# levayz/diffusion_finetuning

Hardware: AMD Instinct MI355X
Metric: images/s SD1.5 LoRA rank-4 512^2 train step (higher is better)
Workload: dtype f16; 1 GPU; SD1.5 UNet-only LoRA rank=4, batch=4/GPU, 512^2 (64x64x4 latents), f16 storage/compute, fp32 accumulate + fp32 master LoRA, full train step (fwd+bwd+clip+AdamW); global_batch=4, parallelism=dp1, lora_params=1246464, overflow=False, hipgraph=True, conv_autotune=True, rccl_ranks=1

## Files before the change

diffusion_finetuning_amd/_native.py:

```python
import ctypes
import os
import threading

import torch

_LIB_PATH = os.environ.get("DFA_LIB_PATH") or os.path.join(os.path.dirname(os.path.abspath(__file__)), "lib", "liblora_hip.so")
_lib = None
_lock = threading.Lock()

ABI_VERSION = 9
PROF_KINDS = 18

_DTYPE_CODE = {torch.float32: 0, torch.float16: 1, torch.bfloat16: 2}

_vp, _i64, _i32, _f32 = ctypes.c_void_p, ctypes.c_int64, ctypes.c_int, ctypes.c_float


class GradProblem(ctypes.Structure):
    _fields_ = [
        ("S", _vp), ("P", _vp), ("out", _vp * 4),
        ("s_stride", _i64), ("p_stride", _i64), ("part_stride", _i64), ("M", _i64),
        ("C", _i32), ("r", _i32), ("rg", _i32), ("out_kn", _i32), ("n_blocks", _i32),
        ("scale", _f32),
    ]
# ... 83 lines not shown
    "lora_adamw_rows": (_i32, [_vp, _vp, _vp, _vp, _vp, _i64, _i32, _vp, _f32, _f32, _f32, _f32, _f32, _f32, _f32, _i32, _vp]),
    "ti_rows_grad": (_i32, [_vp, _vp, _i64, _i32, _vp, _i32, _vp, _i32, _i32, _vp]),
    "ti_rows_adamw_decay": (_i32, [_vp, _i64, _i32, _vp, _i32, _vp, _vp, _vp, _f32, _f32, _f32, _f32, _f32, _f32, _i32, _f32, _f32,
                                   _vp]),
    "geglu_linear_bwd": (_i32, [_vp, _vp, _vp, _vp, _vp, _i64, _i32, _i32, _i32, _vp]),
    "geglu_gate_fwd": (_i32, [_vp, _vp, _i64, _i32, _i32, _vp]),
    "geglu_gate_bwd": (_i32, [_vp, _vp, _vp, _i64, _i32, _i32, _vp]),
    "attn_split_heads": (_i32, [_vp, _vp, _i32, _i32, _i32, _i32, _i32, _i32, _vp]),
    "attn_merge_heads": (_i32, [_vp, _vp, _i32, _i32, _i32, _i32, _i32, _i32, _vp]),
    "attn_merge_heads_strided": (_i32, [_vp, _vp, _i32, _i32, _i32, _i32, _i32, _i64, _i64, _i64, _i32, _vp]),
    "group_norm_act_workspace_bytes": (_i64, [_i32, _i32, _i32, _i32, _i32, _i32]),
    "group_norm_act_plan": (_i32, [_i32, _i32, _i32, _i32, _i32, _i32]),
    "group_norm_act_fwd": (_i32, [_vp] * 8 + [_i32, _i32, _i32, _i32, _f32, _i32, _i32, _i32, _vp]),
    "group_norm_act_bwd": (_i32, [_vp] * 10 + [_i32, _i32, _i32, _i32, _i32, _i32, _i32, _vp]),
    "group_norm_act_bwd_res": (_i32, [_vp] * 11 + [_i32, _i32, _i32, _i32, _i32, _i32, _vp]),
    "residual_bias_add_supported": (_i32, [_i32, _i32, _i32, _i32]),
    "residual_bias_add": (_i32, [_vp] * 5 + [_i32, _i32, _i32, _i32, _vp]),
    "tokens_nchw_supported": (_i32, [_i32, _i32, _i32, _i32]),
    "tokens_to_nchw_add": (_i32, [_vp] * 3 + [_i32, _i32, _i32, _i32, _vp]),
    "nchw_to_tokens": (_i32, [_vp] * 2 + [_i32, _i32, _i32, _i32, _vp]),
    "time_proj_supported": (_i32, [_i32, _i32, _i32]),
    "time_proj_all": (_i32, [_vp] * 6 + [_i32, _i32, _i32, _i32, _vp]),
    "conv3x3_small_supported": (_i32, [_i32, _i32, _i32, _i32, _i32, _i32]),
    "conv3x3_small_workspace_bytes": (_i64, [_i32, _i32, _i32, _i32, _i32, _i32]),
    "conv3x3_small_plan": (_i32, [_i64, _i32, _i32, _i32]),
    "conv3x3_small_plan_channels": (_i32, [_i32, _i32, _i32]),
    "conv3x3_small_pack": (_i32, [_vp, _vp, _i32, _i32, _i32, _i32, _vp]),
    "conv3x3_small": (_i32, [_vp] * 5 + [_i64, _i32, _i32, _i32, _i32, _i32, _i32, _vp]),
    "conv3x3_large_supported": (_i32, [_i32, _i32, _i32, _i32, _i32, _i32]),
    "conv3x3_large_workspace_bytes": (_i64, [_i32, _i32, _i32, _i32, _i32, _i32]),
    "conv3x3_large_plan": (_i32, [_i64, _i32, _i32, _i32]),
    "conv3x3_large_plan_channels": (_i32, [_i32, _i32, _i32]),
    "conv3x3_large": (_i32, [_vp] * 5 + [_i64, _i32, _i32, _i32, _i32, _i32, _i32, _vp]),
    "add_layer_norm_max_channels": (_i32, []),
    "add_layer_norm_fwd": (_i32, [_vp] * 8 + [_i64, _i32, _f32, _i32, _vp]),
    "add_layer_norm_bwd": (_i32, [_vp] * 7 + [_i64, _i32, _i32, _vp]),
    "attn_ctx_supported": (_i32, [_i32, _i32, _i32, _i32, _i32, _i32]),
    "attn_ctx_fwd": (_i32, [_vp, _vp, _vp, _vp, _i32, _i32, _i32, _i32, _i32, _f32, _i32, _vp]),
    "attn_ctx_bwd_workspace_bytes": (_i64, [_i32, _i32, _i32, _i32, _i32]),
    "attn_ctx_fwd_strided": (_i32, [_vp, _vp, _vp, _vp, _i64, _i32, _i32, _i32, _i32, _i32, _f32, _i32, _vp]),
    "attn_ctx_bwd_strided": (_i32, [_vp] * 8 + [_i64, _i64, _i32, _i32, _i32, _i32, _i32, _f32, _i32, _vp]),
    "attn_flash_fwd_strided": (_i32, [_vp, _vp, _vp, _vp, _vp, _i64, _i32, _i32, _i32, _i32, _i32, _f32, _i32, _vp]),
    "attn_flash_bwd_strided": (_i32, [_vp] * 10 + [_i64, _i64, _i32, _i32, _i32, _i32, _i32, _f32, _i32, _vp]),
    "attn_ctx_bwd": (_i32, [_vp, _vp, _vp, _vp, _vp, _vp, _vp, _vp, _i32, _i32, _i32, _i32, _i32, _f32, _i32, _vp]),
    "attn_causal_supported": (_i32, [_i32, _i32, _i32, _i32, _i32]),
    "attn_causal_fwd_strided": (_i32, [_vp, _vp, _vp, _vp, _i64, _i32, _i32, _i32, _i32, _f32, _i32, _vp]),
    "attn_causal_bwd_workspace_bytes": (_i64, [_i32, _i32, _i32, _i32]),
    "attn_causal_bwd_strided": (_i32, [_vp] * 8 + [_i64, _i64, _i32, _i32, _i32, _i32, _f32, _i32, _vp]),
    "attn_flash_supported": (_i32, [_i32, _i32, _i32, _i32, _i32, _i32]),
    "attn_flash_fwd": (_i32, [_vp, _vp, _vp, _vp, _vp, _i32, _i32, _i32, _i32, _i32, _f32, _i32, _vp]),
    "attn_flash_bwd_workspace_bytes": (_i64, [_i32, _i32, _i32]),
    "attn_flash_bwd": (_i32, [_vp] * 10 + [_i32, _i32, _i32, _i32, _i32, _f32, _i32, _vp]),
    "attn_f32_supported": (_i32, [_i32, _i32, _i32, _i32, _i32]),
    "attn_f32_fwd": (_i32, [_vp, _vp, _vp, _vp, _vp, _i32, _i32, _i32, _i32, _i32, _f32, _vp]),
    "attn_f32_bwd_workspace_bytes": (_i64, [_i32, _i32, _i32]),
    "attn_f32_bwd": (_i32, [_vp] * 10 + [_i32, _i32, _i32, _i32, _i32, _f32, _vp]),
    "lora_distill_workspace_bytes": (_i64, [_i64, _i64]),
    "lora_distill_start": (_i32, [_vp, _i32, _i64, _i32, _i64, _vp, _vp]),
    "lora_distill_diff": (_i32, [_vp, _i32, _i64, _i32, _i32, _vp, _vp]),
    "lora_distill_rayleigh_ritz": (_i32, [_vp, _i32, _i32, _i32, ctypes.c_double, _i32, _vp, _vp]),
    "lora_distill_finalize": (_i32, [_vp, _i32, _i32, _f32, _i32, _vp, _vp, _vp]),
    "lora_quantile_clamp": (_i32, [_vp, _i64, _f32, _vp, _vp]),
    "lora_distill_wide_width": (_i32, [_i32]),
    "lora_distill_wide_workspace_bytes": (_i64, [_i64, _i64, _i32]),
    "lora_distill_wide_start": (_i32, [_vp, _i32, _i64, _i32, _i64, _vp, _vp]),
    "lora_distill_wide_diff": (_i32, [_vp, _i32, _i64, _i32, _i32, _i32, _vp, _vp]),
# ... 1153 lines not shown
def conv3x3_small(x, pack, bias, Cout: int):
    _require_device(x, pack, bias)
    N, Cin, H, W = x.shape
    code = dtype_code(x.dtype)
    nbytes = int(lib().conv3x3_small_workspace_bytes(N, Cin, Cout, H, W, code))
    ws = torch.empty(max(nbytes, 16) // 4, dtype=torch.float32, device=x.device)
    y = torch.empty((N, Cout, H, W), dtype=x.dtype, device=x.device)
    _check(lib().conv3x3_small(_ptr(x), _ptr(pack), _ptr(bias), _ptr(y), _ptr(ws), nbytes, N, Cin, Cout, H, W, code, _stream(x)),
           "conv3x3_small")
    return y


def conv3x3_large_supported(N: int, Cin: int, Cout: int, H: int, W: int, dtype) -> bool:
    return dtype in (torch.float16, torch.bfloat16) and bool(lib().conv3x3_large_supported(N, Cin, Cout, H, W, dtype_code(dtype)))


def conv3x3_large_plan(pixels: int, Cin: int, Cout: int, dtype) -> bool:
    return dtype in (torch.float16, torch.bfloat16) and bool(lib().conv3x3_large_plan(int(pixels), Cin, Cout, dtype_code(dtype)))


def conv3x3_large_plan_channels(Cin: int, Cout: int, dtype) -> bool:
    return dtype in (torch.float16, torch.bfloat16) and bool(lib().conv3x3_large_plan_channels(Cin, Cout, dtype_code(dtype)))


def conv3x3_large(x, pack, bias, Cout: int):
    _require_device(x, pack, bias)
    N, Cin, H, W = x.shape
    y = torch.empty((N, Cout, H, W), dtype=x.dtype, device=x.device)
    _check(lib().conv3x3_large(_ptr(x), _ptr(pack), _ptr(bias), _ptr(y), None, 0, N, Cin, Cout, H, W, dtype_code(x.dtype),
                               _stream(x)), "conv3x3_large")
    return y


def tokens_nchw_supported(N: int, C: int, HW: int, dtype) -> bool:
    return dtype in (torch.float16, torch.bfloat16) and bool(lib().tokens_nchw_supported(N, C, HW, dtype_code(dtype)))


def tokens_to_nchw_add(tok, res, shape):
    _require_device(tok, res)
    N, C, H, W = shape
    out = torch.empty(shape, dtype=tok.dtype, device=tok.device)
    _check(lib().tokens_to_nchw_add(_ptr(tok), _ptr(res), _ptr(out), N, C, H * W, dtype_code(tok.dtype), _stream(tok)),
           "tokens_to_nchw_add")
    return out


def nchw_to_tokens(x):
    _require_device(x)
    N, C, H, W = x.shape
    tok = torch.empty((N, H * W, C), dtype=x.dtype, device=x.device)
    _check(lib().nchw_to_tokens(_ptr(x), _ptr(tok), N, C, H * W, dtype_code(x.dtype), _stream(x)), "nchw_to_tokens")
    return tok


def add_layer_norm_supported(x) -> bool:
    C = x.shape[-1] if x.dim() else 0
    return (x.numel() > 0 and x.is_contiguous() and C % 8 == 0 and C <= lib().add_layer_norm_max_channels() and
            x.data_ptr() % 16 == 0)


def add_layer_norm_fwd(x, delta, gamma, beta, eps: float):
    _require_device(x, delta, gamma, beta)
    C = x.shape[-1]
    M = x.numel() // C
    h = None if delta is None else torch.empty_like(x)
    y = torch.empty_like(x)
# ... 262 lines not shown
```

diffusion_finetuning_amd/build_native.py:

```python
import hashlib
import os
import subprocess
import sys
from concurrent.futures import ThreadPoolExecutor

PKG_DIR = os.path.dirname(os.path.abspath(__file__))
CSRC = os.path.join(PKG_DIR, "csrc")
LIB_DIR = os.path.join(PKG_DIR, "lib")
LIB_PATH = os.path.join(LIB_DIR, "liblora_hip.so")
SOURCES = ["lora_gemm.hip", "lora_grad.hip", "ddpm_loss.hip", "optim.hip", "sandwich.hip", "norm.hip", "trunk_edges.hip", "time_proj.hip", "conv_small.hip", "conv_large.hip", "layer_norm.hip", "attn_ctx.hip", "attn_causal.hip", "attn_flash.hip", "attn_f32.hip", "embed.hip", "distill.hip", "distill_wide.hip", "prof.hip"]
HIPCC = os.environ.get("HIPCC", "/opt/rocm/bin/hipcc")
FLAGS = ["--offload-arch=gfx950", "-O3", "-std=c++17", "-fPIC", "-Wall", "-Wno-unused-function"]
SOURCE_FLAGS = {}


def _digest() -> str:
    h = hashlib.sha256()
    for name in sorted(os.listdir(CSRC)) + [os.path.join("..", "..", "include", "lora_hip.h")]:
        with open(os.path.join(CSRC, name), "rb") as f:
            h.update(name.encode())
            h.update(f.read())
    h.update(" ".join(FLAGS).encode())
    for name in sorted(SOURCE_FLAGS):
        h.update((name + " " + " ".join(SOURCE_FLAGS[name])).encode())
    return h.hexdigest()


def build(force: bool = False, verbose: bool = True, variant: str = "", defines=()) -> str:
    os.makedirs(LIB_DIR, exist_ok=True)
    lib_path = os.path.join(LIB_DIR, f"liblora_hip_{variant}.so") if variant else LIB_PATH
    obj_dir = os.path.join(LIB_DIR, f"obj_{variant}") if variant else LIB_DIR
    os.makedirs(obj_dir, exist_ok=True)
    stamp = os.path.join(LIB_DIR, f"liblora_hip_{variant}.stamp" if variant else "liblora_hip.stamp")
    digest = _digest() + (" " + " ".join(defines) if defines else "")
    if not force and os.path.exists(lib_path) and os.path.exists(stamp):
        with open(stamp) as f:
            if f.read().strip() == digest:
                return lib_path

    def compile_one(src: str) -> str:
        obj = os.path.join(obj_dir, src.replace(".hip", ".o"))
        cmd = [HIPCC, *FLAGS, *SOURCE_FLAGS.get(src, []), *defines, "-c", os.path.join(CSRC, src), "-o", obj]
        if verbose:
# ... 24 lines not shown
```

diffusion_finetuning_amd/conv.py:

```python
import torch
import torch.nn as nn
import torch.nn.functional as F
from torch.autograd.function import once_differentiable
from torch.utils.weak import WeakIdKeyDictionary

from . import _native as nat

ROUTES = ("auto", "hip", "large", "stock")

_FAMILY = {"hip": "small", "large": "large"}

_packs = WeakIdKeyDictionary()


def _key(weight):
    return (weight.data_ptr(), weight._version, weight.dtype, weight.device)


def _get_packs(weight):
    entry = _packs.get(weight)
    key = _key(weight)
    if entry is not None and entry[0] == key:
        return entry[1], entry[2]
    if torch.cuda.is_current_stream_capturing():
        return None
    w = weight.detach()
    entry = (key, nat.conv3x3_small_pack(w, False), nat.conv3x3_small_pack(w, True))
    _packs[weight] = entry
    return entry[1], entry[2]


def _weight_eligible(weight, bias) -> bool:
    if not weight.is_cuda or weight.dtype not in (torch.float16, torch.bfloat16) or weight.dim() != 4:
        return False
    if tuple(weight.shape[2:]) != (3, 3) or weight.shape[0] % 32 or weight.shape[1] % 32 or not weight.is_contiguous():
        return False
    if weight.data_ptr() % 16 or weight.requires_grad:
        return False
    if bias is not None and (bias.requires_grad or bias.dtype != weight.dtype or bias.device != weight.device or
                             bias.shape != weight.shape[:1] or not bias.is_contiguous()):
        return False
    return True


def _supported(x, weight, bias, family="small") -> bool:
    if not _weight_eligible(weight, bias):
        return False
    if x.dim() != 4 or x.dtype != weight.dtype or x.device != weight.device or x.shape[1] != weight.shape[1]:
        return False
    if x.numel() == 0 or not x.is_contiguous() or x.data_ptr() % 16:
        return False
    N, Cin, H, W = x.shape
    Cout = weight.shape[0]
    covers = nat.conv3x3_small_supported if family == "small" else nat.conv3x3_large_supported
    return covers(N, Cin, Cout, H, W, x.dtype) and covers(N, Cout, Cin, H, W, x.dtype)


def _run(family, x, pack, bias, Cout):
    return (nat.conv3x3_small if family == "small" else nat.conv3x3_large)(x, pack, bias, Cout)


# ... 18 lines not shown
    def backward(ctx, dy):
        if not ctx.needs_input_grad[0]:
            return (None,) * 7
        dy = dy.contiguous()
        if dy.data_ptr() % 16:
            dy = dy.clone()
        return (_run(ctx.bwd_family, dy, ctx.bwd_pack, None, ctx.cin),) + (None,) * 6


def conv3x3(x: torch.Tensor, weight: torch.Tensor, bias=None, route: str = "auto") -> torch.Tensor:
    if route not in ROUTES:
        raise ValueError(f"conv3x3: route must be one of {ROUTES}, got {route!r}")
    if route != "stock":
        fwd = bwd = None
        if route == "auto":
            if x.dim() == 4 and weight.dim() == 4 and x.is_cuda:
                N, Cin, H, W = x.shape
                fwd = _auto_family(N * H * W, Cin, weight.shape[0], x.dtype)
                bwd = _auto_family(N * H * W, weight.shape[0], Cin, x.dtype) if fwd is not None else None
                if bwd is None or not all(_supported(x, weight, bias, f) for f in {fwd, bwd}):
                    fwd = bwd = None
        elif _supported(x, weight, bias, _FAMILY[route]):
            fwd = bwd = _FAMILY[route]
        packs = _get_packs(weight) if fwd is not None else None
        if packs is not None:
            return _Conv3x3Fn.apply(x, weight, bias, packs[0], packs[1], fwd, bwd)
        if route != "auto":
            raise RuntimeError(f"conv3x3(route={route!r}): the HIP kernel does not cover this call (needs a frozen 16-bit 3×3 "
                               "weight with channel counts that are multiples of 32, an NCHW-contiguous x of the same dtype "
                               "from a 16-byte boundary, and a pack made before stream capture)")
    return F.conv2d(x, weight, bias, padding=1)


def prepack_conv3x3(module: nn.Module, route: str = "auto") -> int:
    if route not in ROUTES:
        raise ValueError(f"prepack_conv3x3: route must be one of {ROUTES}, got {route!r}")
    if route == "stock":
        return 0
    n = 0
    for m in module.modules():
        if type(m) is not nn.Conv2d or m.kernel_size != (3, 3) or m.stride != (1, 1) or m.padding != (1, 1):
            continue
        if m.dilation != (1, 1) or m.groups != 1 or not _weight_eligible(m.weight, m.bias):
            continue
        if route == "auto" and not (nat.conv3x3_small_plan_channels(m.weight.shape[1], m.weight.shape[0], m.weight.dtype) or
                                    nat.conv3x3_large_plan_channels(m.weight.shape[1], m.weight.shape[0], m.weight.dtype)):
            continue
        if _get_packs(m.weight) is not None:
            n += 1
    return n


def packed_bytes() -> int:
    return sum(e[1].numel() * e[1].element_size() + e[2].numel() * e[2].element_size() for e in _packs.values())
```

harness/unet.py:

```python
import math
from dataclasses import dataclass, field
from typing import List, Optional, Tuple

import torch
import torch.nn as nn
import torch.nn.functional as F
from torch.nn.attention import SDPBackend, sdpa_kernel


@dataclass
class UNetConfig:
    in_channels: int = 4
    out_channels: int = 4
    block_out_channels: Tuple[int, ...] = (320, 640, 1280, 1280)
    down_attention: Tuple[bool, ...] = (True, True, True, False)
    layers_per_block: int = 2
    num_heads: Tuple[int, ...] = (8, 8, 8, 8)
    cross_attention_dim: int = 768
    norm_groups: int = 32
    linear_projection: bool = False
    name: str = "sd15"


def sd15_config() -> UNetConfig:
# ... 38 lines not shown
    def forward(self, x):
        return self.linear_2(self.act(self.linear_1(x)))


def _fused_norms(x):
    return x.is_cuda and x.dtype in (torch.float16, torch.bfloat16)


def _norm_act(norm: nn.GroupNorm, x, act: bool, addend=None):
    from diffusion_finetuning_amd.norm import group_norm_act

    return group_norm_act(x, norm.num_groups, norm.weight, norm.bias, norm.eps, act, addend)


def _norm_act_res(norm: nn.GroupNorm, x, act: bool):
    from diffusion_finetuning_amd.norm import group_norm_act_res

    return group_norm_act_res(x, norm.num_groups, norm.weight, norm.bias, norm.eps, act)


def _norm_tokens(norm: nn.GroupNorm, x):
    from diffusion_finetuning_amd.norm import group_norm_tokens

    return group_norm_tokens(x, norm.num_groups, norm.weight, norm.bias, norm.eps)


def _tokens_to_nchw_add(tok, res):
    from diffusion_finetuning_amd.norm import tokens_to_nchw_add

    return tokens_to_nchw_add(tok, res)


CONV3X3_ROUTE = "auto"


def _conv3x3(x, weight, bias=None):
    from diffusion_finetuning_amd.conv import conv3x3

    return conv3x3(x, weight, bias, CONV3X3_ROUTE)


def _residual_bias_add(h, res, b1, b2=None):
    from diffusion_finetuning_amd.norm import residual_bias_add

    return residual_bias_add(h, res, b1, b2)


def _time_projections(temb, layers):
    from diffusion_finetuning_amd.time_proj import time_projections

    return time_projections(temb, layers)


def _layer_norm(norm: nn.LayerNorm, x):
    from diffusion_finetuning_amd import norm as dnorm

    return dnorm.layer_norm(x, norm.weight, norm.bias, norm.eps)


def _add_layer_norm(norm: nn.LayerNorm, x, delta):
    from diffusion_finetuning_amd import norm as dnorm

    return dnorm.add_layer_norm(x, delta, norm.weight, norm.bias, norm.eps)


class ResnetBlock2D(nn.Module):
# ... 139 lines not shown
        x = _norm_act(self.norm, x, False) if _fused_norms(x) else self.norm(x)
        if x.is_cuda and not self.linear_projection:
            x = F.linear(x.permute(0, 2, 3, 1).reshape(b, h * w, c), self.proj_in.weight.view(c, c), self.proj_in.bias)
            for blk in self.transformer_blocks:
                x = blk(x, context)
            x = F.linear(x, self.proj_out.weight.view(c, c), self.proj_out.bias)
            return x.view(b, h, w, c).permute(0, 3, 1, 2).contiguous() + res
        if self.linear_projection:
            x = self.proj_in(x.permute(0, 2, 3, 1).reshape(b, h * w, c))
        else:
            x = self.proj_in(x).permute(0, 2, 3, 1).reshape(b, h * w, c)
        for blk in self.transformer_blocks:
            x = blk(x, context)
        if self.linear_projection:
            x = self.proj_out(x).reshape(b, h, w, c).permute(0, 3, 1, 2).contiguous()
        else:
            x = self.proj_out(x.reshape(b, h, w, c).permute(0, 3, 1, 2))
        return x + res


class Downsample2D(nn.Module):
    def __init__(self, c):
        super().__init__()
        self.conv = nn.Conv2d(c, c, 3, stride=2, padding=1)

    def forward(self, x):
        return self.conv(x)


class Upsample2D(nn.Module):
    def __init__(self, c):
        super().__init__()
        self.conv = nn.Conv2d(c, c, 3, padding=1)

    def forward(self, x):
        x = F.interpolate(x, scale_factor=2.0, mode="nearest")
        if _fused_norms(x) and type(self.conv) is nn.Conv2d:
            return _conv3x3(x, self.conv.weight, self.conv.bias)
        return self.conv(x)


class DownBlock(nn.Module):
    def __init__(self, cin, cout, temb, layers, attn, heads, ctx, groups, linear_proj, add_down):
        super().__init__()
        self.attentions = nn.ModuleList(
            [Transformer2DModel(cout, heads, ctx, groups, linear_proj) for _ in range(layers)] if attn else []
        )
        self.resnets = nn.ModuleList([ResnetBlock2D(cin if i == 0 else cout, cout, temb, groups) for i in range(layers)])
        self.downsamplers = nn.ModuleList([Downsample2D(cout)]) if add_down else None

    def forward(self, x, temb, context, addends=None):
        outs = []
        for i, res in enumerate(self.resnets):
            x = res(x, temb, None if addends is None else addends[i])
            if len(self.attentions):
                x = self.attentions[i](x, context)
            outs.append(x)
        if self.downsamplers is not None:
            x = self.downsamplers[0](x)
            outs.append(x)
        return x, outs


class MidBlock(nn.Module):
    def __init__(self, c, temb, heads, ctx, groups, linear_proj):
        super().__init__()
        self.attentions = nn.ModuleList([Transformer2DModel(c, heads, ctx, groups, linear_proj)])
        self.resnets = nn.ModuleList([ResnetBlock2D(c, c, temb, groups), ResnetBlock2D(c, c, temb, groups)])
# ... 100 lines not shown
```

include/lora_hip.h:

```cpp
#ifndef LORA_HIP_H
#define LORA_HIP_H

#include <stdint.h>

#ifdef __cplusplus
extern "C" {
#endif

#define LORA_HIP_ABI_VERSION 9

enum lora_dtype { LORA_F32 = 0, LORA_F16 = 1, LORA_BF16 = 2 };

enum lora_status {
    LORA_OK = 0,
    LORA_E_BADARG = -1,
    LORA_E_RANK = -2,
    LORA_E_ALIGN = -3,
    LORA_E_LAUNCH = -4,
    LORA_E_UNSUPPORTED = -5
};

int lora_version(void);

const char* lora_status_string(int status);
// ... 202 lines not shown
                       int HW, int groups, int act, int channels_last, int dtype, void* stream);
int group_norm_act_bwd_res(const void* dy, const void* dh , const void* x, const void* addend ,
                           const void* gamma, const void* beta, const float* mean, const float* rstd, void* dx,
                           void* da , void* workspace, int N, int C, int HW, int groups, int act, int dtype,
                           void* stream);

int residual_bias_add_supported(int N, int C, int HW, int dtype);
int residual_bias_add(const void* h, const void* res, const void* b1, const void* b2 , void* out, int N, int C,
                      int HW, int dtype, void* stream);
int tokens_nchw_supported(int N, int C, int HW, int dtype);
int tokens_to_nchw_add(const void* tok, const void* res , void* out, int N, int C, int HW, int dtype,
                       void* stream);
int nchw_to_tokens(const void* x, void* tok, int N, int C, int HW, int dtype, void* stream);

int time_proj_supported(int N, int E, int dtype);
int time_proj_all(const void* t, const void* const* W, const void* const* b , const void* const* cb ,
                  const int* C, void* out, int L, int N, int E, int dtype, void* stream);

int conv3x3_small_supported(int N, int C_in, int C_out, int H, int W, int dtype);
int64_t conv3x3_small_workspace_bytes(int N, int C_in, int C_out, int H, int W, int dtype);
int conv3x3_small_plan(int64_t pixels, int C_in, int C_out, int dtype);
int conv3x3_small_plan_channels(int C_in, int C_out, int dtype);
int conv3x3_small_pack(const void* w, void* packed, int C_in, int C_out, int backward, int dtype, void* stream);
int conv3x3_small(const void* x, const void* wpack, const void* bias , void* y, void* workspace,
                  int64_t workspace_bytes, int N, int C_in, int C_out, int H, int W, int dtype, void* stream);

int conv3x3_large_supported(int N, int C_in, int C_out, int H, int W, int dtype);
int64_t conv3x3_large_workspace_bytes(int N, int C_in, int C_out, int H, int W, int dtype);
int conv3x3_large_plan(int64_t pixels, int C_in, int C_out, int dtype);
int conv3x3_large_plan_channels(int C_in, int C_out, int dtype);
int conv3x3_large(const void* x, const void* wpack, const void* bias , void* y, void* workspace ,
                  int64_t workspace_bytes, int N, int C_in, int C_out, int H, int W, int dtype, void* stream);

int add_layer_norm_max_channels(void);
int add_layer_norm_fwd(const void* x, const void* delta , const void* gamma, const void* beta,
                       void* h , void* y, float* mean, float* rstd, int64_t M, int C, float eps,
                       int dtype, void* stream);
int add_layer_norm_bwd(const void* dy, const void* dh , const void* h, const void* gamma, const float* mean,
                       const float* rstd, void* dx, int64_t M, int C, int dtype, void* stream);

int embed_rows_fwd(const float* table, const int64_t* ids, void* out, int64_t n, int D, int64_t V, int out_dtype, void* stream);
int embed_rows_bwd(const void* dE, const int64_t* ids, float* grad_table, unsigned char* active , int64_t n,
                   int D, int64_t V, int dtype, int accumulate, void* stream);
int lora_adamw_rows(float* param, const float* grad, float* exp_avg, float* exp_avg_sq, const unsigned char* active, int64_t V,
                    int D, const float* norm_in, float grad_mul, float max_norm, float lr, float beta1, float beta2, float eps,
                    float weight_decay, int step, void* stream);

#define LORA_TI_MAX_ROWS 64
int ti_rows_grad(const void* dE, const int64_t* ids, int64_t n, int D, const int64_t* slot_ids, int P, float* grad, int dtype,
                 int accumulate, void* stream);
int ti_rows_adamw_decay(float* table, int64_t V, int D, const int64_t* slot_ids, int P, const float* grad, float* exp_avg,
                        float* exp_avg_sq, float grad_mul, float lr, float beta1, float beta2, float eps, float weight_decay,
                        int step, float decay_lambda, float target_norm, void* stream);

int attn_ctx_supported(int B, int Tq, int Tk, int H, int d, int dtype);
int attn_ctx_fwd_strided(const void* Q, const void* K, const void* V, void* O, int64_t ldk, int B, int Tq, int Tk,
                         int H, int d, float scale, int dtype, void* stream);
int attn_ctx_bwd_strided(const void* Q, const void* K, const void* V, const void* dO, void* dQ, void* dK, void* dV,
                         void* workspace, int64_t ldk, int64_t ld_dk, int B, int Tq, int Tk, int H, int d,
                         float scale, int dtype, void* stream);
int attn_ctx_fwd(const void* Q, const void* K, const void* V, void* O, int B, int Tq, int Tk, int H, int d,
                 float scale, int dtype, void* stream);
int64_t attn_ctx_bwd_workspace_bytes(int B, int Tq, int Tk, int H, int d);
int attn_ctx_bwd(const void* Q, const void* K, const void* V, const void* dO, void* dQ, void* dK, void* dV,
                 void* workspace, int B, int Tq, int Tk, int H, int d, float scale, int dtype, void* stream);

// ... 67 lines not shown
```

Before: 203.2 images/s.

## Fuse nearest 2x upsample with following 3x3 conv via subpixel 2x2 weights

Adds a HIP kernel that computes nearest-upsample followed by a 3x3 conv directly from the low-resolution input. It uses four precombined 2x2 subpixel weight sets, which cuts MACs by about 2.25x and skips materialising the upsampled tensor. A matching backward kernel produces the input gradient at low resolution. The auto route is limited to 640-channel, 4096-pixel upsamplers, so only one SD1.5 upsample layer is covered. It adds a second cached weight pack per eligible conv and a new kernel that needs to be correct.

```diff
diff --git a/diffusion_finetuning_amd/_native.py b/diffusion_finetuning_amd/_native.py
--- a/diffusion_finetuning_amd/_native.py
+++ b/diffusion_finetuning_amd/_native.py
@@ -139,6 +139,11 @@
     "conv3x3_large_plan": (_i32, [_i64, _i32, _i32, _i32]),
     "conv3x3_large_plan_channels": (_i32, [_i32, _i32, _i32]),
     "conv3x3_large": (_i32, [_vp] * 5 + [_i64, _i32, _i32, _i32, _i32, _i32, _i32, _vp]),
+    "conv3x3_up_supported": (_i32, [_i32, _i32, _i32, _i32, _i32, _i32]),
+    "conv3x3_up_plan": (_i32, [_i64, _i32, _i32, _i32]),
+    "conv3x3_up_plan_channels": (_i32, [_i32, _i32, _i32]),
+    "conv3x3_up_pack": (_i32, [_vp, _vp, _i32, _i32, _i32, _i32, _vp]),
+    "conv3x3_up": (_i32, [_vp] * 4 + [_i32, _i32, _i32, _i32, _i32, _i32, _i32, _vp]),
     "add_layer_norm_max_channels": (_i32, []),
     "add_layer_norm_fwd": (_i32, [_vp] * 8 + [_i64, _i32, _f32, _i32, _vp]),
     "add_layer_norm_bwd": (_i32, [_vp] * 7 + [_i64, _i32, _i32, _vp]),
@@ -1358,6 +1363,43 @@
     return y
 
 
+def conv3x3_up_supported(N: int, Cin: int, Cout: int, H: int, W: int, dtype) -> bool:
+    return dtype in (torch.float16, torch.bfloat16) and bool(lib().conv3x3_up_supported(N, Cin, Cout, H, W, dtype_code(dtype)))
+
+
+def conv3x3_up_plan(pixels: int, Cin: int, Cout: int, dtype) -> bool:
+    return dtype in (torch.float16, torch.bfloat16) and bool(lib().conv3x3_up_plan(int(pixels), Cin, Cout, dtype_code(dtype)))
+
+
+def conv3x3_up_plan_channels(Cin: int, Cout: int, dtype) -> bool:
+    return dtype in (torch.float16, torch.bfloat16) and bool(lib().conv3x3_up_plan_channels(Cin, Cout, dtype_code(dtype)))
+
+
+def conv3x3_up_pack(weight, backward: bool):
+    _require_device(weight)
+    Cout, Cin = weight.shape[:2]
+    packed = torch.empty(16 * Cin * Cout, dtype=weight.dtype, device=weight.device)
+    _check(lib().conv3x3_up_pack(_ptr(weight), _ptr(packed), Cin, Cout, int(backward), dtype_code(weight.dtype),
+                                 _stream(weight)), "conv3x3_up_pack")
+    return packed
+
+
+def conv3x3_up(x, pack, bias, Cout: int, backward: bool = False):
+    _require_device(x, pack, bias)
+    N, Cin = x.shape[:2]
+    if backward:
+        if x.shape[2] % 2 or x.shape[3] % 2:
+            raise ValueError("conv3x3_up: the gradient of an upsampled tensor has even height and width")
+        H, W = x.shape[2] // 2, x.shape[3] // 2
+        y = torch.empty((N, Cout, H, W), dtype=x.dtype, device=x.device)
+    else:
+        H, W = x.shape[2:]
+        y = torch.empty((N, Cout, 2 * H, 2 * W), dtype=x.dtype, device=x.device)
+    _check(lib().conv3x3_up(_ptr(x), _ptr(pack), _ptr(None if backward else bias), _ptr(y), N, Cin, Cout, H, W, int(backward),
+                            dtype_code(x.dtype), _stream(x)), "conv3x3_up")
+    return y
+
+
 def tokens_nchw_supported(N: int, C: int, HW: int, dtype) -> bool:
     return dtype in (torch.float16, torch.bfloat16) and bool(lib().tokens_nchw_supported(N, C, HW, dtype_code(dtype)))
 
diff --git a/diffusion_finetuning_amd/build_native.py b/diffusion_finetuning_amd/build_native.py
--- a/diffusion_finetuning_amd/build_native.py
+++ b/diffusion_finetuning_amd/build_native.py
@@ -8,7 +8,7 @@
 CSRC = os.path.join(PKG_DIR, "csrc")
 LIB_DIR = os.path.join(PKG_DIR, "lib")
 LIB_PATH = os.path.join(LIB_DIR, "liblora_hip.so")
-SOURCES = ["lora_gemm.hip", "lora_grad.hip", "ddpm_loss.hip", "optim.hip", "sandwich.hip", "norm.hip", "trunk_edges.hip", "time_proj.hip", "conv_small.hip", "conv_large.hip", "layer_norm.hip", "attn_ctx.hip", "attn_causal.hip", "attn_flash.hip", "attn_f32.hip", "embed.hip", "distill.hip", "distill_wide.hip", "prof.hip"]
+SOURCES = ["lora_gemm.hip", "lora_grad.hip", "ddpm_loss.hip", "optim.hip", "sandwich.hip", "norm.hip", "trunk_edges.hip", "time_proj.hip", "conv_small.hip", "conv_large.hip", "conv_up.hip", "layer_norm.hip", "attn_ctx.hip", "attn_causal.hip", "attn_flash.hip", "attn_f32.hip", "embed.hip", "distill.hip", "distill_wide.hip", "prof.hip"]
 HIPCC = os.environ.get("HIPCC", "/opt/rocm/bin/hipcc")
 FLAGS = ["--offload-arch=gfx950", "-O3", "-std=c++17", "-fPIC", "-Wall", "-Wno-unused-function"]
 SOURCE_FLAGS = {}
diff --git a/diffusion_finetuning_amd/conv.py b/diffusion_finetuning_amd/conv.py
--- a/diffusion_finetuning_amd/conv.py
+++ b/diffusion_finetuning_amd/conv.py
@@ -10,23 +10,27 @@
 
 _FAMILY = {"hip": "small", "large": "large"}
 
+UP_ROUTES = ("auto", "up", "stock")
+
 _packs = WeakIdKeyDictionary()
+_up_packs = WeakIdKeyDictionary()
 
 
 def _key(weight):
     return (weight.data_ptr(), weight._version, weight.dtype, weight.device)
 
 
-def _get_packs(weight):
-    entry = _packs.get(weight)
+def _get_packs(weight, up=False):
+    cache, pack = (_up_packs, nat.conv3x3_up_pack) if up else (_packs, nat.conv3x3_small_pack)
+    entry = cache.get(weight)
     key = _key(weight)
     if entry is not None and entry[0] == key:
         return entry[1], entry[2]
     if torch.cuda.is_current_stream_capturing():
         return None
     w = weight.detach()
-    entry = (key, nat.conv3x3_small_pack(w, False), nat.conv3x3_small_pack(w, True))
-    _packs[weight] = entry
+    entry = (key, pack(w, False), pack(w, True))
+    cache[weight] = entry
     return entry[1], entry[2]
 
 
@@ -111,6 +115,73 @@
     return F.conv2d(x, weight, bias, padding=1)
 
 
+def subpixel_weights(w: torch.Tensor) -> torch.Tensor:
+    G = (((0,), (1, 2)), ((0, 1), (2,)))
+    acc = w.float() if w.dtype in (torch.float16, torch.bfloat16) else w
+    out = acc.new_zeros((2, 2) + tuple(w.shape[:2]) + (2, 2))
+    for a in range(2):
+        for b in range(2):
+            for dr in range(2):
+                for ds in range(2):
+                    total = None
+                    for r in G[a][dr]:
+                        row = None
+                        for s in G[b][ds]:
+                            row = acc[:, :, r, s] if row is None else row + acc[:, :, r, s]
+                        total = row if total is None else total + row
+                    out[a, b, :, :, dr, ds] = total
+    return out.to(w.dtype)
+
+
+class _UpConv3x3Fn(torch.autograd.Function):
+    @staticmethod
+    def forward(ctx, x, weight, bias, fwd_pack, bwd_pack):
+        ctx.bwd_pack = bwd_pack
+        ctx.cin = x.shape[1]
+        return nat.conv3x3_up(x, fwd_pack, bias, weight.shape[0])
+
+    @staticmethod
+    @once_differentiable
+    def backward(ctx, dy):
+        if not ctx.needs_input_grad[0]:
+            return (None,) * 5
+        dy = dy.contiguous()
+        if dy.data_ptr() % 16:
+            dy = dy.clone()
+        return (nat.conv3x3_up(dy, ctx.bwd_pack, None, ctx.cin, backward=True),) + (None,) * 4
+
+
+def _up_supported(x, weight, bias) -> bool:
+    if not _weight_eligible(weight, bias):
+        return False
+    if x.dim() != 4 or x.dtype != weight.dtype or x.device != weight.device or x.shape[1] != weight.shape[1]:
+        return False
+    if x.numel() == 0 or not x.is_contiguous() or x.data_ptr() % 16:
+        return False
+    N, Cin, H, W = x.shape
+    return nat.conv3x3_up_supported(N, Cin, weight.shape[0], H, W, x.dtype)
+
+
+def upsample2x_conv3x3(x: torch.Tensor, weight: torch.Tensor, bias=None, route: str = "auto") -> torch.Tensor:
+    if route not in UP_ROUTES:
+        raise ValueError(f"upsample2x_conv3x3: route must be one of {UP_ROUTES}, got {route!r}")
+    if route != "stock":
+        ok = False
+        if route == "up":
+            ok = _up_supported(x, weight, bias)
+        elif x.dim() == 4 and weight.dim() == 4 and x.is_cuda:
+            N, Cin, H, W = x.shape
+            ok = nat.conv3x3_up_plan(N * H * W, Cin, weight.shape[0], x.dtype) and _up_supported(x, weight, bias)
+        packs = _get_packs(weight, up=True) if ok else None
+        if packs is not None:
+            return _UpConv3x3Fn.apply(x, weight, bias, packs[0], packs[1])
+        if route != "auto":
+            raise RuntimeError("upsample2x_conv3x3(route='up'): the HIP kernel does not cover this call (needs a frozen 16-bit 3×3 "
+                               "weight with channel counts that are multiples of 32, an NCHW-contiguous x of the same dtype "
+                               "from a 16-byte boundary, and a pack made before stream capture)")
+    return conv3x3(F.interpolate(x, scale_factor=2.0, mode="nearest"), weight, bias)
+
+
 def prepack_conv3x3(module: nn.Module, route: str = "auto") -> int:
     if route not in ROUTES:
         raise ValueError(f"prepack_conv3x3: route must be one of {ROUTES}, got {route!r}")
@@ -122,6 +193,9 @@
             continue
         if m.dilation != (1, 1) or m.groups != 1 or not _weight_eligible(m.weight, m.bias):
             continue
+        if route == "auto" and getattr(m, "upsampled_input", False) and nat.conv3x3_up_plan_channels(
+                m.weight.shape[1], m.weight.shape[0], m.weight.dtype):
+            _get_packs(m.weight, up=True)
         if route == "auto" and not (nat.conv3x3_small_plan_channels(m.weight.shape[1], m.weight.shape[0], m.weight.dtype) or
                                     nat.conv3x3_large_plan_channels(m.weight.shape[1], m.weight.shape[0], m.weight.dtype)):
             continue
@@ -131,4 +205,5 @@
 
 
 def packed_bytes() -> int:
-    return sum(e[1].numel() * e[1].element_size() + e[2].numel() * e[2].element_size() for e in _packs.values())
+    return sum(e[1].numel() * e[1].element_size() + e[2].numel() * e[2].element_size()
+               for cache in (_packs, _up_packs) for e in cache.values())
diff --git a/diffusion_finetuning_amd/csrc/conv_up.hip b/diffusion_finetuning_amd/csrc/conv_up.hip
--- /dev/null
+++ b/diffusion_finetuning_amd/csrc/conv_up.hip
@@ -0,0 +1,394 @@
+#include <atomic>
+
+#include "conv_common.h"
+
+namespace {
+
+constexpr int kNTL = 160;
+constexpr int kFragsN = kNTL / 16;
+constexpr int kGroupFrags = 2 * kFragsN;
+constexpr int kWBuf = kGroupFrags * 1024;
+constexpr int kWBufs = 4;
+constexpr int kAhead = 2;
+
+enum Mode { kFwd = 0, kBwd = 2 };
+
+template <int N> __device__ __forceinline__ void wait_barrier() {
+    asm volatile("s_waitcnt vmcnt(%0) lgkmcnt(0)\n\ts_barrier" ::"n"(N) : "memory");
+}
+
+__device__ __forceinline__ void glds16(const void* gsrc, unsigned char* lds_wave_base) {
+    __builtin_amdgcn_global_load_lds((const __attribute__((address_space(1))) void*)(gsrc),
+                                     (__attribute__((address_space(3))) void*)(lds_wave_base), 16, 0, 0);
+}
+
+template <typename T, int MT, int PER, int WM, int MODE>
+__global__ __launch_bounds__(WM * 128) void conv_up_kernel(const T* __restrict__ x, const T* __restrict__ wp,
+                                                           const T* __restrict__ bias, T* __restrict__ y, int Cin, int Cout, int H,
+                                                           int W, int M, int mtiles, int ctiles, int chunks, int Pcap) {
+    using Frag = typename Mfma<T>::Frag;
+    constexpr int NTHR = WM * 128, NW = WM * 2, kPieces = (kGroupFrags + NW - 1) / NW;
+    constexpr int MF = MT / (16 * WM);
+    constexpr int NF = kFragsN / 2;
+    constexpr int NB = MODE == kFwd ? 2 : 1;
+    constexpr int SPC = 2 * NB;
+    extern __shared__ __attribute__((aligned(1024))) unsigned char smem[];
+    unsigned char* const wlds = smem;
+    unsigned char* const alds = smem + kWBufs * kWBuf;
+    const int abytes = Pcap * kPitch;
+    const int tid = threadIdx.x, lane = tid & 63, wave = __builtin_amdgcn_readfirstlane(tid >> 6), wm = wave % WM, wn = wave / WM;
+
+    int mt, nt;
+    {
+        const unsigned total = gridDim.x, id = blockIdx.x;
+        const unsigned q = total >> 3, rem = total & 7, xcd = id & 7, slot = id >> 3;
+        const unsigned n = (xcd < rem ? xcd * (q + 1) : rem * (q + 1) + (xcd - rem) * q) + slot;
+        mt = (int)(n % (unsigned)mtiles);
+        nt = (int)(n / (unsigned)mtiles);
+    }
+    const int ct = nt % ctiles, ta = nt / ctiles;
+
+    const int HW = H * W, W2 = W + 2, PP = (H + 2) * W2;
+    const int m0 = mt * MT;
+    const int q0 = padded_pos(m0, H, W);
+    const int P = tile_positions(m0, MT, M, H, W);
+    const int qlo = q0 - (W2 + 1);
+    const float inv_pp = 1.f / (float)PP, inv_w2 = 1.f / (float)W2, inv_p = 1.f / (float)P;
+    const int CS = MODE == kBwd ? 4 * HW : HW;
+
+    int xoff[PER];
+    int aoff[PER];
+#pragma unroll
+    for (int s = 0; s < PER; ++s) {
+        const int i = tid + s * NTHR, cg = fast_div(i, P, inv_p), p = i - cg * P;
+        const bool unit = cg < 4;
+        const int q = qlo + p, img = fast_div(q, PP, inv_pp), r = q - img * PP, hp = fast_div(r, W2, inv_w2), wq = r - hp * W2;
+        const bool inside = unit && hp >= 1 && hp <= H && wq >= 1 && wq <= W;
+        const int pix = MODE == kBwd ? (hp - 1) * 4 * W + (wq - 1) * 2 : (hp - 1) * W + (wq - 1);
+        xoff[s] = inside ? (img * Cin + cg * 8) * CS + pix : -1;
+        aoff[s] = unit ? p * kPitch + cg * 16 : 2 * abytes + tid * 16;
+    }
+
+    const int nk = MODE == kBwd ? 4 * chunks : chunks;
+    const int c0 = mt % nk;
+    auto kchunk_of = [&](int it) { const int c = c0 + it; return c >= nk ? c - nk : c; };
+    auto phase_of = [&](int kc) { return (kc >= chunks) + (kc >= 2 * chunks) + (kc >= 3 * chunks); };
+
+    T raw[PER][8];
+    auto load_stage = [&](int kc) {
+        const T* base;
+        if (MODE == kBwd) {
+            const int ph = phase_of(kc);
+            base = x + (size_t)(kc - ph * chunks) * kChunk * CS + (ph >> 1) * 2 * W + (ph & 1);
+        } else {
+            base = x + (size_t)kc * kChunk * CS;
+        }
+#pragma unroll
+        for (int s = 0; s < PER; ++s) {
+            const int o = xoff[s] >= 0 ? xoff[s] : 0;
+#pragma unroll
+            for (int c = 0; c < 8; ++c) raw[s][c] = base[o + c * CS];
+        }
+    };
+    auto write_stage = [&](int buf) {
+#pragma unroll
+        for (int s = 0; s < PER; ++s)
+#pragma unroll
+            for (int j = 0; j < 8; ++j) asm volatile("" : "+v"(raw[s][j]));
+#pragma unroll
+        for (int s = 0; s < PER; ++s) {
+            Frag v;
+#pragma unroll
+            for (int j = 0; j < 8; ++j) v[j] = xoff[s] >= 0 ? raw[s][j] : static_cast<T>(0.f);
+            *reinterpret_cast<Frag*>(alds + (aoff[s] < 2 * abytes ? buf * abytes : 0) + aoff[s]) = v;
+        }
+    };
+
+    int lpos[MF];
+    const float inv_hw = 1.f / (float)HW, inv_w = 1.f / (float)W;
+#pragma unroll
+    for (int f = 0; f < MF; ++f) {
+        const int m = min(m0 + wm * (MT / WM) + f * 16 + (lane & 15), M - 1);
+        const int img = fast_div(m, HW, inv_hw), r = m - img * HW, h = fast_div(r, W, inv_w);
+        lpos[f] = (img * PP + (h + 1) * W2 + (r - h * W) + 1 - q0) * kPitch + (lane >> 4) * 16;
+    }
+
+    const int KO = Cout >> 4;
+    const size_t tap_stride = (size_t)KO * 512;
+    auto load_w = [&](int st, int slot, int lo, int hi) {
+        const int kc = kchunk_of(st / SPC), r = st % SPC;
+        const int group = MODE == kBwd ? kc * 4 + r * 2 : (((ta * 2 + (r >> 1)) * chunks + kc) * 4 + (r & 1) * 2);
+        const T* src = wp + (size_t)group * tap_stride + lane * 8;
+        unsigned char* dst = wlds + slot * kWBuf;
+#pragma unroll
+        for (int i = lo; i < hi; ++i) {
+            const int j = min(wave + NW * i, kGroupFrags - 1), t = j / kFragsN, f = j - t * kFragsN;
+            glds16(src + t * tap_stride + (size_t)min(ct * kFragsN + f, KO - 1) * 512, dst + j * 1024);
+        }
+    };
+
+    f32x4 acc[NB][MF][NF];
+#pragma unroll
+    for (int b = 0; b < NB; ++b)
+#pragma unroll
+        for (int f = 0; f < MF; ++f)
+#pragma unroll
+            for (int g = 0; g < NF; ++g) acc[b][f][g] = f32x4{0.f, 0.f, 0.f, 0.f};
+
+    static_assert(kAhead == 2 && kPieces + 8 * PER <= 63, "vmcnt is a 6-bit counter");
+    constexpr int kP1 = (kPieces + 1) / 2;
+    const int steps = nk * SPC;
+    load_stage(c0);
+    load_w(0, 0, 0, kPieces);
+    load_w(1, 1, 0, kPieces);
+    write_stage(0);
+    for (int it = 0; it < nk; ++it) {
+        const unsigned char* ab = alds + (it & 1) * abytes;
+        int wa = ta, wb2 = 0;
+        if (MODE == kBwd) {
+            const int ph = phase_of(kchunk_of(it));
+            wa = ph >> 1, wb2 = ph & 1;
+        }
+#pragma unroll
+        for (int r = 0; r < SPC; ++r) {
+            const int st = it * SPC + r, ahead = min(st + kAhead, steps - 1), slot = st & 3, aslot = (st + kAhead) & 3;
+            if (r == 1) wait_barrier<kPieces + 8 * PER>();
+            else wait_barrier<kPieces>();
+            if (r == SPC - 1) write_stage((it + 1) & 1);
+            load_w(ahead, aslot, 0, kP1);
+            if (r == 0) load_stage(kchunk_of(min(it + 1, nk - 1)));
+            __builtin_amdgcn_sched_barrier(0);
+            const unsigned char* wb = wlds + slot * kWBuf + wn * NF * 1024 + lane * 16;
+            const int bset = MODE == kFwd ? r >> 1 : 0;
+            const int sh0 = MODE == kBwd ? ((2 - wa - r) * W2 + 2 - wb2) * kPitch
+                                         : ((wa + (r & 1)) * W2 + (r >> 1)) * kPitch;
+            const int shd = MODE == kBwd ? -kPitch : kPitch;
+            Frag xf[2][MF], bf[2][NF];
+#pragma unroll
+            for (int f = 0; f < MF; ++f) xf[0][f] = *reinterpret_cast<const Frag*>(ab + lpos[f] + sh0);
+#pragma unroll
+            for (int g = 0; g < NF; ++g) bf[0][g] = *reinterpret_cast<const Frag*>(wb + g * 1024);
+#pragma unroll
+            for (int tt = 0; tt < 2; ++tt) {
+                if (tt == 0) {
+#pragma unroll
+                    for (int f = 0; f < MF; ++f) xf[1][f] = *reinterpret_cast<const Frag*>(ab + lpos[f] + sh0 + shd);
+#pragma unroll
+                    for (int g = 0; g < NF; ++g) bf[1][g] = *reinterpret_cast<const Frag*>(wb + (kFragsN + g) * 1024);
+                }
+#pragma unroll
+                for (int f = 0; f < MF; ++f)
+#pragma unroll
+                    for (int g = 0; g < NF; ++g) acc[bset][f][g] = Mfma<T>::run(xf[tt][f], bf[tt][g], acc[bset][f][g]);
+                if (tt == 0) load_w(ahead, aslot, kP1, kPieces);
+                __builtin_amdgcn_sched_barrier(0);
+            }
+        }
+    }
+
+    asm volatile("s_waitcnt vmcnt(0)" ::: "memory");
+
+#pragma unroll
+    for (int g = 0; g < NF; ++g) {
+        const int k = ct * kNTL + (wn * NF + g) * 16 + (lane & 15);
+        if (k >= Cout) continue;
+        const float b = bias ? to_f32(bias[k]) : 0.f;
+#pragma unroll
+        for (int f = 0; f < MF; ++f) {
+            const int m = m0 + wm * (MT / WM) + f * 16 + (lane >> 4) * 4;
+            if (MODE == kBwd) {
+                struct alignas(8) Out4 { T v[4]; };
+                if ((HW & 3) == 0) {
+                    if (m < M) {
+                        const int img = fast_div(m, HW, inv_hw);
+                        Out4 o;
+#pragma unroll
+                        for (int i = 0; i < 4; ++i) o.v[i] = from_f32<T>(acc[0][f][g][i] + b);
+                        *reinterpret_cast<Out4*>(y + (img * Cout + k) * HW + (m - img * HW)) = o;
+                    }
+                } else {
+#pragma unroll
+                    for (int i = 0; i < 4; ++i)
+                        if (m + i < M) {
+                            const int img = fast_div(m + i, HW, inv_hw);
+                            y[(img * Cout + k) * HW + (m + i - img * HW)] = from_f32<T>(acc[0][f][g][i] + b);
+                        }
+                }
+            } else if ((W & 3) == 0) {
+                struct alignas(16) Out8 { T v[8]; };
+                if (m < M) {
+                    const int img = fast_div(m, HW, inv_hw), r = m - img * HW, h = fast_div(r, W, inv_w), w = r - h * W;
+                    Out8 o;
+#pragma unroll
+                    for (int i = 0; i < 4; ++i) {
+                        o.v[2 * i] = from_f32<T>(acc[0][f][g][i] + b);
+                        o.v[2 * i + 1] = from_f32<T>(acc[NB - 1][f][g][i] + b);
+                    }
+                    *reinterpret_cast<Out8*>(y + ((img * Cout + k) * 2 * H + 2 * h + ta) * 2 * W + 2 * w) = o;
+                }
+            } else {
+#pragma unroll
+                for (int i = 0; i < 4; ++i)
+                    if (m + i < M) {
+                        const int img = fast_div(m + i, HW, inv_hw), r = m + i - img * HW, h = fast_div(r, W, inv_w), w = r - h * W;
+                        T* row = y + ((img * Cout + k) * 2 * H + 2 * h + ta) * 2 * W + 2 * w;
+                        row[0] = from_f32<T>(acc[0][f][g][i] + b);
+                        row[1] = from_f32<T>(acc[NB - 1][f][g][i] + b);
+                    }
+            }
+        }
+    }
+}
+
+template <typename T>
+__global__ __launch_bounds__(256) void conv_up_pack_kernel(const T* __restrict__ w, T* __restrict__ out, int Cin, int Cout,
+                                                           int backward) {
+    const int64_t total = (int64_t)Cin * Cout * 16, o = (int64_t)blockIdx.x * 256 + threadIdx.x;
+    if (o >= total) return;
+    const int Ci = backward ? Cout : Cin, Co = backward ? Cin : Cout, KO = Co >> 4, chunks = Ci >> 5;
+    const int j = (int)(o & 7), l = (int)((o >> 3) & 63);
+    const int64_t rest = o >> 9;
+    const int ko = (int)(rest % KO);
+    const int64_t rest2 = rest / KO;
+    const int t = (int)(rest2 & 3), cc = (int)((rest2 >> 2) % chunks), ph = (int)((rest2 >> 2) / chunks);
+    const int a = ph >> 1, b = ph & 1, dr = t >> 1, ds = t & 1;
+    const int ci = cc * 32 + (l >> 4) * 8 + j, co = ko * 16 + (l & 15);
+    const int k = backward ? ci : co, c = backward ? co : ci;
+    const int rlo = dr ? 1 + a : 0, rhi = dr ? 2 : a, slo = ds ? 1 + b : 0, shi = ds ? 2 : b;
+    const T* src = w + ((int64_t)k * Cin + c) * 9;
+    float sum = 0.f;
+    for (int r = rlo; r <= rhi; ++r) {
+        float row = 0.f;
+        for (int s = slo; s <= shi; ++s) row += to_f32(src[r * 3 + s]);
+        sum += row;
+    }
+    out[o] = from_f32<T>(sum);
+}
+
+struct UGeo {
+    int MT = 0, per = 0, mtiles = 0, ctiles = 0, ntiles = 0, chunks = 0, Pcap = 0, M = 0;
+    bool ok = false;
+};
+
+constexpr int kVariants = 3;
+constexpr int kVarMT[kVariants] = {128, 64, 64};
+constexpr int kVarPer[kVariants] = {3, 3, 6};
+constexpr int kVarWM[kVariants] = {4, 2, 2};
+
+int max_positions(int MT, int M, int H, int W) {
+    const int HW = H * W, mtiles = (M + MT - 1) / MT;
+    int a = MT, b = HW;
+    while (b) { const int c = a % b; a = b, b = c; }
+    const int period = HW / a;
+    int pmax = 0;
+    for (int t = 0; t < mtiles && t < period; ++t) {
+        const int p = tile_positions(t * MT, MT, M, H, W);
+        pmax = p > pmax ? p : pmax;
+    }
+    return pmax;
+}
+
+UGeo up_geo(int N, int Cin, int Cout, int H, int W, int mode) {
+    UGeo g;
+    if (!conv_shape_in_range(N, Cin, Cout, H, W)) return g;
+    const int64_t M64 = (int64_t)N * H * W;
+    if (4 * M64 * (mode == kBwd ? Cin : Cout) >= (1ll << 31)) return g;
+    const int M = N * H * W, ctiles = (Cout + kNTL - 1) / kNTL, ntiles = ctiles * (mode == kFwd ? 2 : 1);
+    const int p128 = max_positions(128, M, H, W), p64 = max_positions(64, M, H, W);
+    const bool fits[kVariants] = {p128 <= 32 * kVarWM[0] * kVarPer[0], p64 <= 32 * kVarWM[1] * kVarPer[1],
+                                  p64 <= 32 * kVarWM[2] * kVarPer[2]};
+    int v = -1;
+    if (fits[0] && (int64_t)((M + 127) / 128) * ntiles >= kCUs) v = 0;
+    else if (fits[1]) v = 1;
+    else if (fits[2]) v = 2;
+    if (v < 0) return g;
+    g.MT = kVarMT[v], g.per = kVarPer[v], g.Pcap = v == 0 ? p128 : p64;
+    g.mtiles = (M + g.MT - 1) / g.MT, g.ctiles = ctiles, g.ntiles = ntiles, g.chunks = Cin / kChunk, g.M = M;
+    g.ok = (int64_t)g.mtiles * g.ntiles <= (1 << 20);
+    return g;
+}
+
+template <typename T, int MT, int PER, int WM, int MODE>
+bool launch_up(const T* x, const T* wp, const T* bias, T* y, int Cin, int Cout, int H, int W, const UGeo& g, hipStream_t s) {
+    const int lds = kWBufs * kWBuf + 2 * g.Pcap * kPitch + WM * 128 * 16;
+    auto kern = conv_up_kernel<T, MT, PER, WM, MODE>;
+    static std::atomic<int> lds_allowed{0};
+    if (lds > lds_allowed.load(std::memory_order_relaxed)) {
+        if (hipFuncSetAttribute(reinterpret_cast<const void*>(kern), hipFuncAttributeMaxDynamicSharedMemorySize, lds) != hipSuccess)
+            return false;
+        lds_allowed.store(lds, std::memory_order_relaxed);
+    }
+    hipLaunchKernelGGL(kern, dim3(g.mtiles * g.ntiles), dim3(WM * 128), lds, s, x, wp, bias, y, Cin, Cout, H, W, g.M, g.mtiles,
+                       g.ctiles, g.chunks, g.Pcap);
+    return true;
+}
+
+template <typename T, int MODE>
+int run_up(const void* x_, const void* wp_, const void* bias_, void* y_, int Cin, int Cout, int H, int W, const UGeo& g,
+           hipStream_t s) {
+    const T *x = static_cast<const T*>(x_), *wp = static_cast<const T*>(wp_), *bias = static_cast<const T*>(bias_);
+    T* y = static_cast<T*>(y_);
+    const bool ok = g.MT == 128   ? launch_up<T, 128, 3, 4, MODE>(x, wp, bias, y, Cin, Cout, H, W, g, s)
+                    : g.per == 3 ? launch_up<T, 64, 3, 2, MODE>(x, wp, bias, y, Cin, Cout, H, W, g, s)
+                                 : launch_up<T, 64, 6, 2, MODE>(x, wp, bias, y, Cin, Cout, H, W, g, s);
+    if (!ok) return LORA_E_LAUNCH;
+    LORA_LAUNCH_CHECK();
+    return LORA_OK;
+}
+
+
+bool up_plan_channels(int C, int64_t pixels ) {
+    return C == 640 && (pixels == 4096 || pixels == 0);
+}
+
+}
+
+extern "C" int conv3x3_up_supported(int N, int C_in, int C_out, int H, int W, int dtype) {
+    return (dtype == LORA_F16 || dtype == LORA_BF16) && up_geo(N, C_in, C_out, H, W, kFwd).ok &&
+                   up_geo(N, C_out, C_in, H, W, kBwd).ok
+               ? 1 : 0;
+}
+
+extern "C" int conv3x3_up_plan(int64_t pixels, int C_in, int C_out, int dtype) {
+    if (dtype != LORA_F16 && dtype != LORA_BF16) return 0;
+    return pixels >= 1 && C_in == C_out && up_plan_channels(C_in, pixels) ? 1 : 0;
+}
+
+extern "C" int conv3x3_up_plan_channels(int C_in, int C_out, int dtype) {
+    if (dtype != LORA_F16 && dtype != LORA_BF16) return 0;
+    return C_in == C_out && up_plan_channels(C_in, 0) ? 1 : 0;
+}
+
+extern "C" int conv3x3_up_pack(const void* w, void* packed, int C_in, int C_out, int backward, int dtype, void* stream) {
+    if (!w || !packed || C_in < 1 || C_out < 1 || (backward != 0 && backward != 1)) return LORA_E_BADARG;
+    if (dtype != LORA_F16 && dtype != LORA_BF16) return dtype == LORA_F32 ? LORA_E_UNSUPPORTED : LORA_E_BADARG;
+    if (C_in % 32 || C_out % 32 || (int64_t)C_in * C_out * 16 >= (1ll << 31)) return LORA_E_UNSUPPORTED;
+    if (!aligned16(packed)) return LORA_E_ALIGN;
+    hipStream_t s = static_cast<hipStream_t>(stream);
+    const int64_t total = (int64_t)C_in * C_out * 16;
+    const dim3 grid((unsigned)((total + 255) / 256));
+    if (dtype == LORA_F16)
+        hipLaunchKernelGGL(conv_up_pack_kernel<half_t>, grid, dim3(256), 0, s, static_cast<const half_t*>(w),
+                           static_cast<half_t*>(packed), C_in, C_out, backward);
+    else
+        hipLaunchKernelGGL(conv_up_pack_kernel<bf16_t>, grid, dim3(256), 0, s, static_cast<const bf16_t*>(w),
+                           static_cast<bf16_t*>(packed), C_in, C_out, backward);
+    LORA_LAUNCH_CHECK();
+    return LORA_OK;
+}
+
+extern "C" int conv3x3_up(const void* x, const void* wpack, const void* bias, void* y, int N, int C_in, int C_out, int H, int W,
+                          int backward, int dtype, void* stream) {
+    if (!x || !wpack || !y || N < 1 || C_in < 1 || C_out < 1 || H < 1 || W < 1 || (backward != 0 && backward != 1))
+        return LORA_E_BADARG;
+    if (dtype != LORA_F16 && dtype != LORA_BF16) return dtype == LORA_F32 ? LORA_E_UNSUPPORTED : LORA_E_BADARG;
+    const UGeo g = up_geo(N, C_in, C_out, H, W, backward ? kBwd : kFwd);
+    if (!g.ok) return LORA_E_UNSUPPORTED;
+    if (!aligned16(x) || !aligned16(wpack) || !aligned16(y)) return LORA_E_ALIGN;
+    hipStream_t s = static_cast<hipStream_t>(stream);
+    if (backward)
+        return dtype == LORA_F16 ? run_up<half_t, kBwd>(x, wpack, nullptr, y, C_in, C_out, H, W, g, s)
+                                 : run_up<bf16_t, kBwd>(x, wpack, nullptr, y, C_in, C_out, H, W, g, s);
+    return dtype == LORA_F16 ? run_up<half_t, kFwd>(x, wpack, bias, y, C_in, C_out, H, W, g, s)
+                             : run_up<bf16_t, kFwd>(x, wpack, bias, y, C_in, C_out, H, W, g, s);
+}
diff --git a/harness/unet.py b/harness/unet.py
--- a/harness/unet.py
+++ b/harness/unet.py
@@ -94,6 +94,7 @@
 
 
 CONV3X3_ROUTE = "auto"
+UPSAMPLE_ROUTE = "auto"
 
 
 def _conv3x3(x, weight, bias=None):
@@ -299,8 +300,13 @@
     def __init__(self, c):
         super().__init__()
         self.conv = nn.Conv2d(c, c, 3, padding=1)
+        self.conv.upsampled_input = True
 
     def forward(self, x):
+        if _fused_norms(x) and type(self.conv) is nn.Conv2d and (CONV3X3_ROUTE == "auto" or UPSAMPLE_ROUTE != "auto"):
+            from diffusion_finetuning_amd.conv import upsample2x_conv3x3
+
+            return upsample2x_conv3x3(x, self.conv.weight, self.conv.bias, UPSAMPLE_ROUTE)
         x = F.interpolate(x, scale_factor=2.0, mode="nearest")
         if _fused_norms(x) and type(self.conv) is nn.Conv2d:
             return _conv3x3(x, self.conv.weight, self.conv.bias)
diff --git a/include/lora_hip.h b/include/lora_hip.h
--- a/include/lora_hip.h
+++ b/include/lora_hip.h
@@ -258,6 +258,13 @@
 int conv3x3_large(const void* x, const void* wpack, const void* bias , void* y, void* workspace ,
                   int64_t workspace_bytes, int N, int C_in, int C_out, int H, int W, int dtype, void* stream);
 
+int conv3x3_up_supported(int N, int C_in, int C_out, int H, int W, int dtype);
+int conv3x3_up_plan(int64_t pixels, int C_in, int C_out, int dtype);
+int conv3x3_up_plan_channels(int C_in, int C_out, int dtype);
+int conv3x3_up_pack(const void* w, void* packed, int C_in, int C_out, int backward, int dtype, void* stream);
+int conv3x3_up(const void* x, const void* wpack, const void* bias , void* y, int N, int C_in, int C_out, int H, int W,
+               int backward, int dtype, void* stream);
+
 int add_layer_norm_max_channels(void);
 int add_layer_norm_fwd(const void* x, const void* delta , const void* gamma, const void* beta,
                        void* h , void* y, float* mean, float* rstd, int64_t M, int C, float eps,
```

Measured after the change: 204.3 images/s (median of 6 runs). About the same (+0.5%).
